# antofuller/jumbo_mae_tpu

Hardware: AMD Instinct MI355X
Metric: pretrain images/sec (whole node) ViT-L/16 224 mask75% at 1/2/4/8 MI355X (higher is better)
Workload: dtype bf16; 1 GPU; model=vit_large_patch16 jumbo-MAE (3 CLS, shared jumbo MLP) + decoder 8x512x16h, global_batch=4096, seq_len=52, decoder_seq_len=199, parallelism=dp1, per_gpu_batch=4096, grad_accum=2, micro_batch=2048, grad_ckpt=False, hip_graph=False, optimizer=adamw(0.9,0.95) wd0.05 warmup-cosine

## Files before the change

### jumbo_mae_tpu_amd/csrc/bindings.cpp

```cpp
#include <torch/extension.h>
#include <c10/hip/HIPStream.h>
#include <hip/hip_runtime.h>

#include <array>
#include <climits>

#include "jm_api.h"

namespace {

hipStream_t stream() { return c10::hip::getCurrentHIPStream().stream(); }

#define CHECK_CUDA(x) TORCH_CHECK((x).is_cuda(), #x " must be a GPU tensor")
#define CHECK_CONTIG(x) TORCH_CHECK((x).is_contiguous(), #x " must be contiguous")
#define CHECK_DT(x, d) TORCH_CHECK((x).scalar_type() == (d), #x " has wrong dtype")

const uint16_t* bf(const torch::Tensor& t) { return reinterpret_cast<const uint16_t*>(t.data_ptr()); }
uint16_t* bfm(torch::Tensor& t) { return reinterpret_cast<uint16_t*>(t.data_ptr()); }
uint16_t* bfp(const torch::Tensor& t) { return reinterpret_cast<uint16_t*>(t.data_ptr()); }
const float* fopt(const c10::optional<torch::Tensor>& t) {
  return t.has_value() && t->defined() ? t->data_ptr<float>() : nullptr;
}
float* fopt_m(c10::optional<torch::Tensor>& t) { return t.has_value() && t->defined() ? t->data_ptr<float>() : nullptr; }

// ... 767 lines not shown
  GemmEpi ep{nullptr, nullptr, N};
  ep.part = out.data_ptr<float>();
  run_nt("gemm_nt_f32", jm_gemm_nt_plan(M, N, K, EPI_PARTIAL, A.stride(0), 1), A, B, ep);
  return out;
}

torch::Tensor gemm_nt_dgelu(torch::Tensor A, torch::Tensor B, torch::Tensor pre, c10::optional<torch::Tensor> dbias,
                            bool deriv, double rate) {
  CHECK_DT(pre, deriv ? torch::kUInt8 : torch::kBFloat16);
  const auto [M, N, K] = check_nt_operands("gemm_nt_dgelu", A, B);
  TORCH_CHECK(pre.is_contiguous() && pre.size(0) == M && pre.size(1) == N, "gemm_nt_dgelu: pre [M,N]");
  auto out = torch::empty({M, N}, A.options());
  GemmEpi ep{nullptr, bfm(out), N};
  if (deriv) {
    ep.dqa = pre.data_ptr<uint8_t>();
    ep.dqs = (rate > 0.0 ? keep_params(rate).second : 1.f) / GD_Q;
  } else {
    ep.aux = bf(pre);
  }
  GemmPlan plan = jm_gemm_nt_plan(M, N, K, deriv ? EPI_DMUL : EPI_DGELU, A.stride(0), 1);
  float* db = bias_ptr("gemm_nt_dgelu dbias", dbias, N);
  torch::Tensor part;
  if (db) {
    const auto f32 = A.options().dtype(torch::kFloat32);
    part = plan.colpart_zero ? torch::zeros({plan.colpart_rows, N}, f32) : torch::empty({plan.colpart_rows, N}, f32);
    ep.colpart = part.data_ptr<float>();
  } else {
    plan.colpart = false;
  }
  run_nt("gemm_nt_dgelu", plan, A, B, ep);
  if (db) check_rc(jm_splitk_reduce_add(part.data_ptr<float>(), db, N, plan.colpart_rows, stream()),
                   "gemm_nt_dgelu dbias");
  return out;
}

py::dict gemm_nt_plan_dict(int M, int N, int K, int epi, long lda, int splits) {
  const GemmPlan p = jm_gemm_nt_plan(M, N, K, epi, lda, splits);
  using namespace py::literals;
  return py::dict("status"_a = p.status, "family"_a = p.family, "tile_rows"_a = p.tile_rows,
                  "tile_cols"_a = p.tile_cols, "row_tiles"_a = p.row_tiles, "col_tiles"_a = p.col_tiles,
                  "tiles"_a = p.tiles, "grid"_a = p.grid, "tail_S"_a = p.tail_S, "tail_r"_a = p.tail_r,
                  "tail_floats"_a = p.tail_floats, "colpart"_a = p.colpart, "colpart_rows"_a = p.colpart_rows,
                  "colpart_zero"_a = p.colpart_zero);
}

torch::Tensor rrc_resize(torch::Tensor src, torch::Tensor tab, int64_t size, int64_t tmp_bytes, int64_t tmp_rows_max) {
  CHECK_CUDA(src);
  CHECK_CUDA(tab);
  CHECK_DT(src, torch::kUInt8);
  CHECK_DT(tab, torch::kInt64);
  TORCH_CHECK(src.dim() == 1 && src.is_contiguous(), "rrc_resize: src must be a flat uint8 buffer");
  TORCH_CHECK(tab.dim() == 2 && tab.size(1) == 13 && tab.is_contiguous(), "rrc_resize: tab [B, 13] int64");
  TORCH_CHECK(size > 0 && size <= 4096 && tmp_bytes > 0 && tmp_rows_max > 0, "rrc_resize: bad sizes");
  const int B = tab.size(0);
  auto out = torch::empty({B, 3, size, size}, src.options());
  auto tmp = torch::empty({tmp_bytes}, src.options());
  check_rc(jm_rrc_resize(src.data_ptr<uint8_t>(), tab.data_ptr<int64_t>(), B, (int)size, tmp.data_ptr<uint8_t>(),
                         (int)tmp_rows_max, out.data_ptr<uint8_t>(), stream()),
           "rrc_resize");
  return out;
}

torch::Tensor window_resize(torch::Tensor src, torch::Tensor tab, int64_t size, int64_t tmp_bytes,
                            int64_t tmp_rows_max) {
  CHECK_CUDA(src);
  CHECK_CUDA(tab);
// ... 1177 lines not shown
  m.def("attn_dropout", &attn_dropout, py::arg("S"), py::arg("hd"));
  m.def("gemm_tn_wgrad", &gemm_tn_wgrad, py::arg("dy"), py::arg("x"), py::arg("g"), py::arg("store") = false);
  m.def("gemm_tn_wgrad_seg", &gemm_tn_wgrad_seg, py::arg("dys"), py::arg("xs"), py::arg("g"), py::arg("store") = false);
  m.def("zero_ranges", &zero_ranges, "zero float ranges of a flat buffer (one launch)");
  m.def("colsum_add_f32", &colsum_add_f32, "g += x.sum(0) for a row-strided fp32 [rows, n] view");
  m.def("gemm_tn_wgrad_seg_group", &gemm_tn_wgrad_seg_group, py::arg("dys"), py::arg("xs"), py::arg("gs"),
        py::arg("stores") = std::vector<bool>{}, "grouped segmented weight gradients (<= 2 problems)");
  m.def("gemm_tn_wgrad_group", &gemm_tn_wgrad_group, py::arg("dys"), py::arg("xs"), py::arg("gs"),
        py::arg("stores") = std::vector<bool>{}, "grouped weight gradients over one M (<= 4 problems)");
  m.def("gemm_test_force", &jm_gemm_test_force, py::arg("path"), py::arg("rows") = 0,
        "numerics tests only: NT GEMM kernel path 0 = by shape, 1 = 64-deep main loop everywhere, "
        "2 = 4-phase kernels at every M without tail split (rows = forced tile height)");
  m.def("gemm_nt_plan", &gemm_nt_plan_dict, py::arg("M"), py::arg("N"), py::arg("K"), py::arg("epi") = 0,
        py::arg("lda") = 0, py::arg("splits") = 1,
        "the launch plan of an NT GEMM (csrc/gemm_plan.h GemmPlan) as a dict; read-only");
  m.def(
      "gemm_nt_tiles", [](int M, int N, int K, int epi, long lda) { return jm_gemm_nt_plan(M, N, K, epi, lda, 1).tiles; },
      py::arg("M"), py::arg("N"), py::arg("K") = 1024, py::arg("epi") = 0, py::arg("lda") = 0,
      "output tiles (workgroups before split-K) of an NT launch");
  m.def(
      "gemm_nt_tail_plan",
      [](int M, int N, int K, int epi, long lda) {
        const GemmPlan p = jm_gemm_nt_plan(M, N, K, epi, lda, 1);
        return std::make_pair(p.tail_S, p.tail_r);
      },
      py::arg("M"), py::arg("N"), py::arg("K"), py::arg("epi") = 0, py::arg("lda") = 0,
      "(S, tail tiles) of the tail split of an NT launch (S = 0: none); read-only");
  m.def("transpose_bf16_batch", &transpose_bf16_batch);
  m.def("gemm_nt_splitk", &gemm_nt_splitk, py::arg("A"), py::arg("B"), py::arg("bias") = py::none(),
        py::arg("splits") = 8, py::arg("add") = py::none());
  m.def("gemm_nt_dgelu", &gemm_nt_dgelu, py::arg("A"), py::arg("B"), py::arg("pre"), py::arg("dbias") = py::none(),
        py::arg("deriv") = false, py::arg("rate") = 0.0);
  m.def("gemm_nt_f32", &gemm_nt_f32, py::arg("A"), py::arg("B"));
  m.def("gemm_nt", &gemm_nt, py::arg("A"), py::arg("B"), py::arg("bias") = py::none(), py::arg("gelu") = false,
        py::arg("gelu_only") = false, py::arg("gelu_deriv") = false, py::arg("seed") = py::none(),
        py::arg("rate") = 0.0);
  m.def("opt_sumsq", &opt_sumsq);
  m.def("opt_adamw", &opt_adamw);
  m.def("opt_lamb_phase1", &opt_lamb_phase1);
  m.def("opt_lars_norms", &opt_lars_norms);
  m.def("opt_apply_trust", &opt_apply_trust);
  m.def("opt_sgd", &opt_sgd);
  m.def("opt_ema", &opt_ema, py::arg("master"), py::arg("ema"), py::arg("rows"), py::arg("meta"),
        py::arg("ema_hyper"));
  m.def("ema_swap", &ema_swap, py::arg("master"), py::arg("ema"), py::arg("shadow"), py::arg("rows"));
  m.def("opt_seg_stats", &opt_seg_stats, py::arg("master"), py::arg("grad"), py::arg("p_old"), py::arg("rows"),
        py::arg("meta"), py::arg("out") = py::none());
  m.def("patchify_normalize", &patchify_normalize);
  m.def("gather_patches", &gather_patches);
  m.def("embed_finish", &embed_finish);
  m.def("zero_f32", &zero_f32, "fp32 zero fill kernel (the store-mode gradients' pre-reduce fill)");
  m.def("mask_ids", &mask_ids, "random-masking permutation ids + mask from noise (one workgroup per row)");
  m.def("unshuffle_fwd", &unshuffle_fwd);
  m.def("unshuffle_bwd", &unshuffle_bwd);
  m.def("patch_mse_fwd", &patch_mse_fwd);
  m.def("mix_patches", &mix_patches);
  m.def("patch_mse_bwd", &patch_mse_bwd);
  m.def("recon", &recon, py::arg("pred"), py::arg("images"), py::arg("mask"), py::arg("p"), py::arg("norm_pix"),
        py::arg("fill") = 127, py::arg("out") = py::none(),
        "MAE reconstruction panels -> (recon, paste, masked uint8 [B, 3, H, W], err fp32 [B, N])");
  m.def("cls_loss_fwd", &cls_loss_fwd, py::arg("logits"), py::arg("labels"), py::arg("perm") = py::none(),
        py::arg("w") = py::none(), py::arg("smoothing") = 0.0, py::arg("mode") = 0);
  m.def("cls_loss_bwd", &cls_loss_bwd, py::arg("dloss"), py::arg("logits"), py::arg("labels"),
        py::arg("perm"), py::arg("w"), py::arg("smoothing"), py::arg("mode"), py::arg("lse"));
  m.def("kd_loss_fwd", &kd_loss_fwd, py::arg("z"), py::arg("u"), py::arg("temperature") = 1.0, py::arg("mode") = 0,
        "distillation loss -> (kd fp32 [B], agree bool [B], lse fp32 [B, 4], t int32 [B])");
// ... 65 lines not shown
```

### jumbo_mae_tpu_amd/csrc/gemm.hip

```cpp
#include <type_traits>

#include "common.h"
#include "jm_api.h"

namespace {

constexpr int BM = 256, BN = 256;
constexpr size_t GEMM_SMEM = 128 * 1024;

typedef __attribute__((address_space(3))) void lds_void_t;

JM_DEVICE __amdgpu_buffer_rsrc_t make_rsrc(const uint16_t* base, long bytes) {
  const int n = bytes >= 0xffffffffL ? -1 : (int)bytes;
  return __builtin_amdgcn_make_buffer_rsrc((void*)base, (short)0, n, 0x00020000);
}

JM_DEVICE void blds16(__amdgpu_buffer_rsrc_t r, uint32_t voff, uint32_t soff, uint16_t* l) {
  __builtin_amdgcn_raw_ptr_buffer_load_lds(r, (lds_void_t*)(l), 16, voff, soff, 0, 0);
}

JM_DEVICE bf16x8_t lds8(const uint16_t* p) { return *reinterpret_cast<const bf16x8_t*>(p); }

JM_DEVICE f32x4_t mfma16(bf16x8_t a, bf16x8_t b, f32x4_t c) {
  return __builtin_amdgcn_mfma_f32_16x16x32_bf16(a, b, c, 0, 0, 0);
// ... 51 lines not shown
            gd_put<3>(dv[3], gd_put<2>(dv[2], gd_put<1>(dv[1], gd_put<0>(dv[0], 0u))));
        store4(ep.out2 + (long)m * ep.ldo + n, gv);
        continue;
      }
      store4(ep.out + (long)m * ep.ldo + n, v);
      if (EPI == EPI_GELU) {
        float gv[4];
#pragma unroll
        for (int i = 0; i < 4; ++i) gv[i] = gelu_tanh_f(bf2f(f2bf(v[i])));
        store4(ep.out2 + (long)m * ep.ldo + n, gv);
      }
    }
  }
}

template <int BNT = BN, int TR = BM>
JM_DEVICE void tile_of(int M, int N, int GROUP_M, int& m0, int& n0, int splits = 1, int* split = nullptr) {
  const int nM = (M + TR - 1) / TR, nN = (N + BNT - 1) / BNT;
  const int nwg = nM * nN * splits;
  const int orig = blockIdx.x;
  const int xcd = orig & 7, q = nwg >> 3, r = nwg & 7;
  int wg = (xcd < r ? xcd * (q + 1) : r * (q + 1) + (xcd - r) * q) + (orig >> 3);
  if (split) {
    *split = wg / (nM * nN);
    wg -= *split * (nM * nN);
  }
  const int per_group = GROUP_M * nN;
  const int first_m = (wg / per_group) * GROUP_M;
  const int gsz = min(nM - first_m, GROUP_M);
  m0 = (first_m + (wg % per_group) % gsz) * TR;
  n0 = ((wg % per_group) / gsz) * BNT;
}

JM_DEVICE void tile_coords(int g, int M, int N, int GROUP_M, int& m0, int& n0) {
  const int nM = (M + BM - 1) / BM, nN = (N + BN - 1) / BN;
  const int per_group = GROUP_M * nN;
  const int first_m = (g / per_group) * GROUP_M;
  const int gsz = min(nM - first_m, GROUP_M);
  m0 = (first_m + (g % per_group) % gsz) * BM;
  n0 = ((g % per_group) / gsz) * BN;
}

JM_DEVICE void tile_of_range(int M, int N, int GROUP_M, int t_begin, int t_count, int splits, int& m0, int& n0,
                             int& split, int& tg) {
  const int nwg = t_count * splits;
  const int orig = blockIdx.x;
  const int xcd = orig & 7, q = nwg >> 3, r = nwg & 7;
  int wg = (xcd < r ? xcd * (q + 1) : r * (q + 1) + (xcd - r) * q) + (orig >> 3);
  split = wg / t_count;
  tg = wg - split * t_count;
  tile_coords(t_begin + tg, M, N, GROUP_M, m0, n0);
}

template <typename T>
JM_DEVICE void st16(T* p, uint4 v, bool nts) {
  typedef __attribute__((ext_vector_type(4))) unsigned int u32x4_t;
  if (nts) __builtin_nontemporal_store(u32x4_t{v.x, v.y, v.z, v.w}, reinterpret_cast<u32x4_t*>(p));
  else *reinterpret_cast<uint4*>(p) = v;
}

JM_DEVICE void st8(uint8_t* p, uint2 v, bool nts) {
  typedef __attribute__((ext_vector_type(2))) unsigned int u32x2_t;
  if (nts) __builtin_nontemporal_store(u32x2_t{v.x, v.y}, reinterpret_cast<u32x2_t*>(p));
  else *reinterpret_cast<uint2*>(p) = v;
}

JM_DEVICE uint4 pack8(const float* f) {
  uint4 v;
  v.x = pack_bf2(f[0], f[1]);
  v.y = pack_bf2(f[2], f[3]);
  v.z = pack_bf2(f[4], f[5]);
  v.w = pack_bf2(f[6], f[7]);
// ... 488 lines not shown
  } else if (N % 8 == 0)
    epilogue_lds<EPI, NTW, 512, BN, true, 2 * HR>(acc, ep, smem, M, N, m0, n0, wr, wc, l16, g);
  else
    epilogue<EPI, NTW, MTW>(acc, ep, M, N, m0 + wr * HR, n0 + wc * NTW * 16, l16, g);
}

template <int EPI, int MTL = 4>
__global__ __launch_bounds__(512, 1) void gemm_p4_kernel(const uint16_t* __restrict__ A, long lda,
                                                         const uint16_t* __restrict__ B, long ldb, int M, int N,
                                                         int K, GemmEpi ep, int GROUP_M) {
  JM_DGUARD(blockDim.x == 512 && K % 128 == 0 && M > 0 && N > 0);
  extern __shared__ __attribute__((aligned(16))) uint16_t smem[];
  if (__builtin_amdgcn_readfirstlane(threadIdx.x) >= 256) __builtin_amdgcn_s_setprio(1);
  int m0, n0, split = 0;
  if (EPI != EPI_PARTIAL && ep.t_count > 0) {
    int tg;
    tile_of_range(M, N, GROUP_M, ep.t_begin, ep.t_count, 1, m0, n0, split, tg);
  } else {
    tile_of<BN, 128 + 32 * MTL>(M, N, GROUP_M, m0, n0, EPI == EPI_PARTIAL ? ep.splits : 1,
                                EPI == EPI_PARTIAL ? &split : nullptr);
  }
  int k_begin = 0;
  if (EPI == EPI_PARTIAL) {
    const int ku = K / 128;
    const int ku0 = split * ku / ep.splits, ku1 = (split + 1) * ku / ep.splits;
    k_begin = ku0 * 128;
    K = (ku1 - ku0) * 128;
  }
  f32x4_t acc[8][4];
  p4_mainloop<MTL>(A, lda, B, ldb, M, N, m0, n0, k_begin, K, acc, smem);
  p4_epilogue<EPI, MTL>(acc, ep, M, N, m0, n0, split, smem);
}

constexpr int NBM = 128, NBN = 192, NKT = 64;
constexpr int N_AEL = NBM * NKT, N_BEL = NBN * NKT, N_STAGE = N_AEL + N_BEL;
constexpr int N_RING = 3;
constexpr int N_LD = NBN + 8;
static_assert(N_RING * N_STAGE * 2 <= (int)GEMM_SMEM, "narrow ring exceeds the LDS budget");

JM_DEVICE void narrow_tile(int M, int N, int GROUP_M, int splits, int& m0, int& n0, int& split) {
  const int nM = (M + NBM - 1) / NBM, nN = (N + NBN - 1) / NBN;
  const int tiles = nM * nN, nwg = tiles * splits;
  const int orig = blockIdx.x;
  const int xcd = orig & 7, q = nwg >> 3, r = nwg & 7;
  int wg = (xcd < r ? xcd * (q + 1) : r * (q + 1) + (xcd - r) * q) + (orig >> 3);
  split = wg / tiles;
  wg -= split * tiles;
  const int per_group = GROUP_M * nN;
  const int first_m = (wg / per_group) * GROUP_M;
  const int gsz = min(nM - first_m, GROUP_M);
  m0 = (first_m + (wg % per_group) % gsz) * NBM;
  n0 = ((wg % per_group) / gsz) * NBN;
}

template <int EPI>
JM_DEVICE void narrow_epilogue(const f32x4_t (&acc)[4][3], const GemmEpi& ep, uint16_t* cs, int M, int N, int m0,
                               int n0, int split, int wr, int wc, int l16, int g) {
  if constexpr (EPI == EPI_PARTIAL) {
    float* dst = ep.part + (long)split * M * N;
#pragma unroll
    for (int mt = 0; mt < 4; ++mt) {
      const int m = m0 + wr * 64 + mt * 16 + l16;
      if (m >= M) continue;
#pragma unroll
      for (int nt = 0; nt < 3; ++nt) {
        const int n = n0 + wc * 48 + nt * 16 + 4 * g;
// ... 330 lines not shown
  g_test_path = (path == 1 || path == 2) ? path : 0;
  g_test_rows = (g_test_path == 2 && (rows == 224 || rows == 192 || rows == 160 || rows == 256)) ? rows : 0;
}

GemmPlan jm_gemm_nt_plan(int M, int N, int K, int epi, long lda, int splits) {
  return gemm_nt_plan(M, N, K, epi, lda, splits, num_cus(), g_test_path, g_test_rows);
}

int jm_gemm_nt(const GemmPlan& p, const uint16_t* A, const uint16_t* B, long ldb, const GemmEpi& ep, hipStream_t st) {
  if (p.status) return p.status;
  if ((long)p.N * ldb * 2 >= (1L << 32)) return -2;
  if ((p.tail_S && ep.tail == nullptr) || p.colpart != (ep.colpart != nullptr)) return -5;
  return with_epi(p.epi, [&](auto e) {
    constexpr int EPI = decltype(e)::value;
    GemmEpi em = ep;
    em.splits = p.splits;
    em.tail_S = p.tail_S;
    em.t_begin = 0;
    em.t_count = p.tail_S ? p.grid : 0;
    launch_main<EPI>(p, A, B, ldb, em, st);
    if constexpr (gemm_tail_epi(EPI)) {
      if (p.tail_S) {
        GemmEpi et = em;
        et.t_begin = p.grid;
        et.t_count = p.tail_r;
        launch<gemm_nt64_kernel<EPI_TAIL, false>>(GEMM_SMEM, p.tail_r * p.tail_S, p, A, B, ldb, et, st);
        tail_finish_kernel<EPI><<<p.tail_r * GEMM_PLAN_TAIL_BANDS, 256, 0, st>>>(et, p.M, p.N, GEMM_GROUP);
      }
    }
    return 0;
  });
}

JM_DEBUG_EXPORT(gemm)
```

### jumbo_mae_tpu_amd/csrc/gemm_plan.h

```cpp
#pragma once
#include <initializer_list>

enum { EPI_STORE = 0, EPI_GELU = 1, EPI_DGELU = 2, EPI_PARTIAL = 3, EPI_GELU_ONLY = 4, EPI_TAIL = 5, EPI_GELU_D = 6,
       EPI_DMUL = 7 };

enum { GEMM_NARROW = 0,
       GEMM_P4 = 1,
       GEMM_NT64 = 2 };

constexpr int GEMM_PLAN_BM = 256, GEMM_PLAN_BN = 256, GEMM_PLAN_NBM = 128, GEMM_PLAN_NBN = 192;
constexpr int GEMM_PLAN_TAIL_BANDS = 8;

constexpr bool gemm_tail_epi(int epi) {
  return epi == EPI_STORE || epi == EPI_GELU || epi == EPI_DGELU || epi == EPI_GELU_ONLY;
}

struct GemmPlan {
  int status;
  int M, N, K, epi, splits;
  long lda;
  int family;
  int tile_rows, tile_cols;
  int row_tiles, col_tiles, tiles;
  int grid;
// ... 48 lines not shown
    if (S > K / 512) S = K / 512;
    if (S > 8) S = 8;
    if (S < 2) S = 0, r = 0;
  }

  int rows = BM;
  if (!narrow && deep && !splitk && (long)M * lda * 2 < (1L << 31) - (1L << 20)) {
    if (force_rows) {
      rows = force_rows;
    } else {
      float best_c = S ? (t256 / ncu + 0.8f) * BM : (float)cdiv(t256, ncu) * BM;
      for (int tr : {224, 192, 160}) {
        const float c = (float)cdiv(cdiv(M, tr) * nN, ncu) * tr * gemm_rows_cost(tr);
        if (c < best_c) best_c = c, rows = tr;
      }
    }
  }
  if (rows != BM) S = 0, r = 0;

  p.family = narrow ? GEMM_NARROW : (deep && (epi != EPI_PARTIAL || K / 128 >= splits) ? GEMM_P4 : GEMM_NT64);
  p.tile_rows = narrow ? NBM : rows;
  p.tile_cols = narrow ? NBN : BN;
  p.row_tiles = (int)cdiv(M, p.tile_rows);
  p.col_tiles = (int)cdiv(N, p.tile_cols);
  p.tiles = p.row_tiles * p.col_tiles;
  p.grid = epi == EPI_PARTIAL ? p.tiles * splits : p.tiles - r;
  p.tail_S = S, p.tail_r = r;
  p.tail_floats = (long)S * r * BM * BN;
  p.colpart = colsum;
  p.colpart_rows = p.row_tiles + GEMM_PLAN_TAIL_BANDS * r;
  p.colpart_zero = r > 0;
  return p;
}
```

### jumbo_mae_tpu_amd/csrc/jm_api.h

```cpp
#pragma once
#include <cstddef>
#include <cstdint>

#include <hip/hip_runtime.h>

#include "gemm_plan.h"

struct JmDrop {
  const int64_t* seed;
  uint32_t thr;
  float scale;
  long ioff;
};

struct JmLnRes {
  const uint16_t* y;
  uint16_t* dy;
  long yB, yT;
  const float* scale;
  const float* mask;
  int T0;
  float* dscale;
  float* dbias;
  JmDrop drop;
// ... 8 lines not shown
  int tile0[5];
  int n;
};

struct TnSegs {
  const uint16_t* a[64];
  const uint16_t* b[64];
  int rows;
  int n;
};

constexpr float GD_Q = 195.f;
constexpr int GD_Z = 34;

struct GemmEpi {
  const float* bias;
  uint16_t* out;
  long ldo;
  uint16_t* out2;
  const uint16_t* aux;
  float* colpart;
  float* part;
  int splits;
  float* tail;
  int tail_S;
  int t_begin;
  int t_count;
  const int64_t* dseed;
  uint32_t dthr;
  float dscale;
  uint8_t* dq;
  const uint8_t* dqa;
  float dqs;
};


int jm_layernorm_fwd(const float* x, long sB, long sT, int B, int T, int D, const float* gamma, const float* beta,
                     float eps, void* y, int out_bf16, float* mean, float* rstd, hipStream_t st, uint16_t* y2 = nullptr);
int jm_layernorm_bwd(const void* dy, int dy_bf16, const float* x, long sB, long sT, int B, int T, int D,
                     const float* mean, const float* rstd, const float* gamma, float* dx_ptr, long oB, long oT,
                     const float* dres, long rB, long rT, float* dgamma, float* dbeta, int accum_params, float* ws,
                     const JmLnRes* res, hipStream_t st, const uint16_t* hx = nullptr,
                     const float* beta = nullptr);
int jm_layernorm_bwd_blocks(int rows, int D);
int jm_residual_ln_fwd(const float* x, long sB, long sT, const uint16_t* y, const float* scale, const float* mask,
                       float* x1, long oB, long oT, uint16_t* h, float* mean, float* rstd, int B, int T, int T0,
                       int D, const float* gamma, const float* beta, float eps, hipStream_t st, int R0 = 0,
                       JmDrop drop = JmDrop{nullptr, 0u, 1.f, 0});
int jm_debug_line_layernorm();

int jm_gelu_fwd(const uint16_t* h, uint16_t* a, long n, hipStream_t st);
long jm_rowcol_ws_floats(int M, int N, int nacc);
int jm_gelu_bwd(const uint16_t* h, const uint16_t* da, uint16_t* dh, float* bias_grad, int M, int N, hipStream_t st,
                int deriv, float* ws);
int jm_colsum_bf16(const uint16_t* x, float* acc, int M, int N, hipStream_t st, float* ws);
int jm_residual_fwd(const float* x, long sB, long sT, int B, int T, int D, const uint16_t* y, const float* scale,
                    const float* mask, float* out, long oB, long oT, hipStream_t st, JmDrop drop);
int jm_residual_bwd(const float* dout, long dB, long dT, const uint16_t* y, const float* scale, const float* mask,
                    float* dscale, uint16_t* dy, int B, int T, int D, float* dbias, long yB, long yT, hipStream_t st,
                    JmDrop drop, float* ws);
void jm_zero_f32(float* p, long n, hipStream_t st);
int jm_splitk_reduce_add(const float* part, float* g, long n, int S, hipStream_t st, int store = 0);
int jm_colsum_add_f32(const float* x, long ld, int rows, long n, float* g, hipStream_t st);
int jm_zero_ranges(float* base, const long long* desc, int n, long long blocks, hipStream_t st);
int jm_transpose_bf16(const uint16_t* src, uint16_t* dst, int R, int C, hipStream_t st);
int jm_transpose_bf16_batch(const long long* desc, int n, int tiles, hipStream_t st);
// ... 37 lines not shown
void jm_ema_swap(float* p, float* ema, uint16_t* shadow, const int* chunks, int nchunks, long n, hipStream_t st);
constexpr int JM_SEG_STATS_COLS = 7;
void jm_opt_seg_stats(const float* p, const float* g, const float* p_old, const int* chunks, int nchunks,
                      const float* meta, int nseg, long n, double* part, double* out, hipStream_t st);
int jm_debug_line_optim();

int jm_patchify_normalize(const uint8_t* img, float* out, int B, int H, int W, int p, hipStream_t st);
int jm_gather_patches(const uint8_t* img, const int* ids, long idsB, uint16_t* out, int B, int K, int H, int W, int p,
                      hipStream_t st);
int jm_embed_finish(const uint16_t* e, const float* pos, const int* ids, long idsB, const float* cls, float* out,
                    int B, int C, int K, int D, hipStream_t st);
int jm_mask_ids(const float* noise, int R, int N, int keep, int64_t* shuffle, int64_t* restore, int* keep32,
                int* restore32, float* mask, hipStream_t st);
int jm_unshuffle_fwd(const uint16_t* y, const float* tok, const int* restore, long rsB, const float* pos, float* out,
                     int B, int C, int K, int N, int d, hipStream_t st);
int jm_unshuffle_bwd_blocks(int B, int C, int N, int rows_per_block);
int jm_unshuffle_bwd(const float* dout, const int* restore, long rsB, uint16_t* dy, double* part, int B, int C, int K,
                     int N, int d, int rows_per_block, hipStream_t st);
int jm_mix_patches(const uint8_t* img, const int* perm, const float* prm, const int* box, uint16_t* out, int B, int H,
                   int W, int p, hipStream_t st);
int jm_patch_mse_fwd(const uint16_t* pred, long ldp, const uint8_t* img, float* mse, long rows, int N, int H, int W,
                     int p, int norm_pix, hipStream_t st);
int jm_patch_mse_bwd(const uint16_t* pred, long ldp, const uint8_t* img, const float* dmse, uint16_t* dpred, long rows,
                     int N, int H, int W, int p, int norm_pix, hipStream_t st);
int jm_debug_line_mae();

int jm_recon(const void* pred, int pred_bf16, const uint8_t* img, const float* mask, long maskB, uint8_t* recon,
             uint8_t* paste, uint8_t* masked, float* err, int B, int H, int W, int p, int norm_pix, int fill,
             hipStream_t st);
int jm_debug_line_recon();

GemmPlan jm_gemm_nt_plan(int M, int N, int K, int epi, long lda, int splits);
int jm_gemm_nt(const GemmPlan& plan, const uint16_t* A, const uint16_t* B, long ldb, const GemmEpi& ep, hipStream_t st);
void jm_gemm_test_force(int path, int rows);
int jm_debug_line_gemm();

size_t jm_gemm_tn_smem();
int jm_gemm_tn_plan(const TnGroup& grp, int M, int* S_out);
int jm_gemm_tn(const TnGroup& grp, const TnSegs* segs, int M, int sps, int S, hipStream_t st, int store);
int jm_debug_line_gemm_tn();

int jm_dropout_apply(const void* x, void* y, long n, int bf16, const int64_t* seed, uint32_t thr, float scale,
                     hipStream_t st);
int jm_gelu_drop(const uint16_t* h, uint16_t* g, uint16_t* gp, long n, const int64_t* seed, uint32_t thr, float scale,
                 hipStream_t st);
int jm_softmax_dropout_fwd(const float* z, float* p, float* pd, long rows, int S, const int64_t* seed, uint32_t thr,
                           float scale, hipStream_t st);
int jm_softmax_dropout_bwd(const float* dpd, const float* p, float* dz, long rows, int S, const int64_t* seed,
                           uint32_t thr, float scale, hipStream_t st);
int jm_debug_line_dropout();

int jm_rrc_resize(const uint8_t* src, const int64_t* tab, int B, int S, uint8_t* tmp, int tmp_rows_max, uint8_t* out,
                  hipStream_t st);
int jm_window_resize(const uint8_t* src, const int64_t* tab, int B, int S, uint8_t* tmp, int tmp_rows_max,
                     uint8_t* out, hipStream_t st);
int jm_window_tab();
int jm_rrc_kmax();
int jm_debug_line_augment();

int jm_aug_stat_words();
int jm_aug_record_len();
int jm_aug_chain(uint8_t* images, uint8_t* scratch, const double* chain, int B, int slots, int S, uint32_t* stats,
                 hipStream_t st);
int jm_augmix_mix(const uint8_t* orig, const uint8_t* chains, const float* table, uint8_t* out, int B, int W, int S,
                  int blended, hipStream_t st);
int jm_erase_paste(uint8_t* images, const int64_t* table, const uint8_t* fill, long fill_len, int B, int S,
// ... 89 lines not shown
```

### jumbo_mae_tpu_amd/ops/blocks.py

```python

from __future__ import annotations


import torch

from typing import NamedTuple

from . import attn_maps as AM
from . import attn_stats as AS
from . import dropout as Dr
from . import prims as P


LINKS = True
FWD_LINKS = True


class Link:

    __slots__ = ("spec", "dy", "done", "dx_key", "ln1", "h1")

    def __init__(self, ln1=None):
        self.spec = None
        self.dy = None
# ... 44 lines not shown
    if AS._COLLECTOR is not None:
        AS.observe(qkv.view(B, S, -1), attn.heads)
    if AM._COLLECTOR is not None:
        AM.observe(qkv.view(B, S, -1), attn.heads)
    o, lse = P.attn_fwd(qkv.view(B, S, -1), attn.heads, drop=(dr.attn, dr.rate) if dr is not None else None)
    a = P.linear_fwd(o.view(B * S, -1), attn.wo_k, attn.wo_b)
    return qkv, o, lse, a, qs


def _od(dr: Drops | None, name: str, base):
    return None if dr is None else (getattr(dr, name), dr.rate, base)


def _attn_bwd(attn, da, h1, qkv, o, lse, B, S, wo_bias_done=False, dr: Drops | None = None, rope=None, qs=None):
    do = P.linear_bwd(da, o.view(B * S, -1), attn.wo_k, attn.wo_b, bias_done=wo_bias_done)
    plain = rope is None and qs is None
    dqkv, bd = P.attn_bwd(do, qkv.view(B, S, -1), o, lse, attn.heads, attn.qkv_b if plain else None,
                          drop=(dr.attn, dr.rate) if dr is not None else None)
    if qs is not None:
        dqkv, dg = P.qknorm_bwd_(dqkv.view(B, S, -1), qs, attn.heads, attn.q_norm.master, attn.k_norm.master, rope)
        attn.q_norm.accumulate_grad(dg[0])
        attn.k_norm.accumulate_grad(dg[1])
    elif rope is not None:
        dqkv = P.rope_(dqkv.view(B, S, -1), attn.heads, rope.n_cls, rope.gw, rope.table, rope.pos, inverse=True)
    return P.linear_bwd(dqkv.view(B * S, -1), h1, attn.qkv_k, attn.qkv_b, bias_done=bd)


def _ff_fwd(ff, h, train=True, rate=0.0, sh=None, so=None):
    if ff.kind == "swiglu":
        pre = P.linear_fwd(h, ff.w13.k, ff.w13.b)
        a = P.swiglu_fwd(pre, (sh, rate) if sh is not None else None)
        y = P.linear_fwd(a, ff.w2.k, ff.w2.b)
        return pre, a, y, False
    pre, g, deriv, dropped = P.linear_gelu_fwd_saved(h, ff.w1.k, ff.w1.b, need_pre=train,
                                                     drop=(sh, rate) if sh is not None else None)
    if sh is not None and not dropped:
        g, pre = Dr.gelu_drop(pre, None, sh, rate)
        deriv = True
    y = P.linear_fwd(g, ff.w2.k, ff.w2.b)
    return pre, g, y, deriv


def _ff_bwd(ff, dy, h, pre, g, w2_bias_done=False, dx_add=None, deriv=False, rate=0.0, sh=None):
    if ff.kind == "swiglu":
        da = P.linear_bwd(dy, g, ff.w2.k, ff.w2.b, bias_done=w2_bias_done)
        hb13 = ff.w13.b if ff.w13.k.segs[0].trainable else None
        dpre, bias_done = P.swiglu_bwd(pre, da, hb13, (sh, rate) if sh is not None else None)
        return P.linear_bwd(dpre, h, ff.w13.k, ff.w13.b, bias_done=bias_done, dx_add=dx_add)
    hb1 = ff.w1.b if ff.w1.k.segs[0].trainable else None
    dpre, bias_done = P.linear_gelu_bwd(dy, g, pre, ff.w2.k, ff.w2.b, hb1, w2_bias_done, deriv, rate)
    return P.linear_bwd(dpre, h, ff.w1.k, ff.w1.b, bias_done=bias_done, dx_add=dx_add)


def _note_uses(*handles):
    for h in handles:
        if h is not None:
            h.note_use()


def _attn_handles(attn):
    return (attn.qkv_k, attn.qkv_b, attn.wo_k, attn.wo_b, attn.q_norm, attn.k_norm)


def _ff_handles(ff):
    if ff.kind == "swiglu":
        return (ff.w13.k, ff.w13.b, ff.w2.k, ff.w2.b)
    return (ff.w1.k, ff.w1.b, ff.w2.k, ff.w2.b)


class JumboBlockFn(torch.autograd.Function):
    @staticmethod
    def forward(ctx, x, anchor, layer, m1, m2, m3, link_in, link_out, train=True, dr=None, rope=None):
        B, S, D = x.shape
        C = layer.C
        J = C * D
        dt = layer.norm1.g.store.compute_dtype
        h1, mu1, rs1 = _ln1_fwd(x, layer, link_in, dt)
        qkv, o, lse, a, qs = _attn_fwd(layer.attn, h1, B, S, dr, rope)
        x1, hp, mup, rsp = P.residual_ln_fwd(x, a, layer.scale1, m1, layer.norm2.g, layer.norm2.b, C,
                                             drop=_od(dr, "wo", a))
        cls_in = x1[:, :C].reshape(B, 1, J)
        hc, muc, rsc, hcb = P.ln_fwd(cls_in, layer.norm3.g, layer.norm3.b, torch.float32, dt)
        rate = dr.rate if dr is not None else 0.0
        jpre, jg, jy, jd = _ff_fwd(layer.jumbo_mlp, hcb, train, rate, dr and dr.jh, dr and dr.jo)
        pin = x1[:, C:]
        fpre, fg, fy, fd = _ff_fwd(layer.ff, hp, train, rate, dr and dr.fh, dr and dr.fo)
        x2 = torch.empty_like(x1)
        P.residual_fwd(hc.view(B, 1, J), jy, layer.scale3, m3, out=x2[:, :C].reshape(B, 1, J), drop=_od(dr, "jo", jy))
        nl = link_out.ln1 if link_out is not None else None
        if nl is not None:
            _, h1n, mun, rsn = P.residual_ln_fwd(x1, fy, layer.scale2, m2, nl[0], nl[1], 0, C, out=x2,
                                                 drop=_od(dr, "fo", fy))
            link_out.put_h1(x2, h1n, mun, rsn)
        else:
            P.residual_fwd(pin, fy, layer.scale2, m2, out=x2[:, C:], drop=_od(dr, "fo", fy))
        ctx.save_for_backward(x, mu1, rs1, h1, qkv, o, lse, a, x1, muc, rsc, hcb, jpre, jg, jy,
                              hp, mup, rsp, fpre, fg, fy, m1, m2, m3, qs)
        ctx.layer = layer
        ctx.link_in, ctx.link_out = link_in, link_out
        ctx.gelu_deriv = (jd, fd)
        ctx.gelu_rate = rate
        ctx.dr = dr
        ctx.rope = rope
        if link_out is not None:
            link_out.spec = P.ResSpec(fy, layer.scale2, m2, layer.ff.w2.b, C, drop=_od(dr, "fo", fy))
        return x2

    @staticmethod
    def backward(ctx, dx2):
        with P.paired_wgrads():
            dx = _jumbo_bwd(ctx, dx2)
        return dx, None, None, None, None, None, None, None, None, None, None


def _jumbo_bwd(ctx, dx2):
    (x, mu1, rs1, h1, qkv, o, lse, a, x1, muc, rsc, hcb, jpre, jg, jy,
     hp, mup, rsp, fpre, fg, fy, m1, m2, m3, qs) = ctx.saved_tensors
    layer = ctx.layer
    dr = ctx.dr
# ... 119 lines not shown
```

### jumbo_mae_tpu_amd/ops/prims.py

```python

from __future__ import annotations

import contextlib
import math
import os

from typing import NamedTuple

import torch
import torch.nn.functional as F

from ..models.params import Handle
from . import _ext
from . import qknorm as QN
from . import swiglu as SG
from .rope import rope_torch

LN_EPS = 1e-6
_GELU_C = math.sqrt(2.0 / math.pi)


def hip(t: torch.Tensor) -> bool:
    return _ext.use_hip(t)

# ... 97 lines not shown

_GEMM_MODE = "auto"
_DGRAD_OURS = True
_CLS_LOSS_OURS = True
_KD_OURS = True
_EVAL_REPORT_OURS = True
_BN_OURS = True
_KNN_OURS = True
_FEAT_STATS_OURS = True
_NORMS_OURS = True
_ATTN_STATS_OURS = True
_ATTN_MAPS_OURS = True
_ROPE_OURS = True
_QKNORM_OURS = True
_SWIGLU_OURS = True


NARROW_MAX_M = 4096
_NARROW_FUSED_MIN_TILES = 160


def nt_tiles(M: int, N: int) -> int:
    if M < NARROW_MAX_M:
        return -(-M // 128) * -(-N // 192)
    return -(-M // 256) * -(-N // 256)


def use_our_gemm(M: int, N: int, K: int, fused_gelu: bool = False) -> bool:
    if _GEMM_MODE == "blas" or K % 64 or N % 8:
        return False
    if M >= NARROW_MAX_M:
        return True
    return not fused_gelu or nt_tiles(M, N) >= _NARROW_FUSED_MIN_TILES


def splitk_plan(M: int, N: int, K: int) -> int:
    if _GEMM_MODE == "blas" or M >= NARROW_MAX_M or K % 64 or N % 8:
        return 0
    if nt_tiles(M, N) >= _NARROW_FUSED_MIN_TILES:
        return 0
    s = min(256 // nt_tiles(M, N), K // 512, 16)
    return s if s >= 2 else 0


def _pad_cols(t: torch.Tensor, mult: int = 64) -> torch.Tensor:
    c = t.shape[1]
    pad = -c % mult
    return F.pad(t, (0, pad)) if pad else t.contiguous()


def linear_fwd(x2: torch.Tensor, hw: Handle, hb: Handle | None) -> torch.Tensor:
    w = hw.weight()
    if hip(x2) and x2.dtype == torch.bfloat16:
        s = splitk_plan(x2.shape[0], w.shape[0], x2.shape[1])
        if s:
            return _ext.load().gemm_nt_splitk(x2, w, hb.master if hb is not None else None, s)
    if hip(x2) and x2.dtype == torch.bfloat16 and use_our_gemm(x2.shape[0], w.shape[0], x2.shape[1]):
        return _ext.load().gemm_nt(x2, w, hb.master if hb is not None else None, False)[0]
    if hb is not None:
        return torch.addmm(hb.weight(), x2, w.t())
    return x2 @ w.t()


def linear_gelu_fwd(x2: torch.Tensor, hw: Handle, hb: Handle | None, need_pre: bool = True):
    w = hw.weight()
    if hip(x2) and x2.dtype == torch.bfloat16 and use_our_gemm(x2.shape[0], w.shape[0], x2.shape[1], True):
# ... 577 lines not shown
```

Before: 6652 images/sec.

## Run jumbo-MLP and patch-MLP GEMMs together in one grouped NT launch

Adds a grouped GEMM kernel that runs two independent NT problems, the small jumbo CLS MLP and the large per-patch MLP, in a single launch with one shared tile size and an XCD-aware workgroup remap. Both the first (GELU-derivative) and second (store) FFN GEMMs in the block forward go through it when one problem is below the narrow-M threshold and the other is above. The aim is to fill the GPU with the small jumbo GEMM's tiles alongside the large one instead of running an under-occupied launch on its own. The cost is a single row-tile size for both problems and extra epilogue selection per workgroup.

```diff
diff --git a/jumbo_mae_tpu_amd/csrc/bindings.cpp b/jumbo_mae_tpu_amd/csrc/bindings.cpp
--- a/jumbo_mae_tpu_amd/csrc/bindings.cpp
+++ b/jumbo_mae_tpu_amd/csrc/bindings.cpp
@@ -823,6 +823,102 @@
   if (db) check_rc(jm_splitk_reduce_add(part.data_ptr<float>(), db, N, plan.colpart_rows, stream()),
                    "gemm_nt_dgelu dbias");
   return out;
+}
+
+using OptTensors = std::vector<c10::optional<torch::Tensor>>;
+std::vector<torch::Tensor> gemm_nt_group(std::vector<torch::Tensor> A, std::vector<torch::Tensor> B, OptTensors bias,
+                                         int64_t epi, OptTensors aux, OptTensors dbias, OptTensors seed, double rate,
+                                         OptTensors out, OptTensors out2) {
+  TORCH_CHECK(A.size() == 2 && B.size() == 2, "gemm_nt_group: two problems");
+  TORCH_CHECK(epi == EPI_STORE || epi == EPI_GELU_D || epi == EPI_DMUL, "gemm_nt_group: epilogue");
+  const auto opt = [](const OptTensors& v, int p, const char* what) -> const torch::Tensor* {
+    TORCH_CHECK(v.empty() || v.size() == 2, "gemm_nt_group: ", what, " must be empty or have two entries");
+    return !v.empty() && v[p].has_value() && v[p]->defined() ? &*v[p] : nullptr;
+  };
+  NtGroup grp{};
+  std::vector<torch::Tensor> res, part(2);
+  for (int p = 0; p < 2; ++p) {
+    const auto [M, N, K] = check_nt_operands("gemm_nt_group", A[p], B[p]);
+    TORCH_CHECK(epi == EPI_STORE || N % 8 == 0, "gemm_nt_group: N % 8 == 0 with a fused epilogue");
+    NtProblem& q = grp.p[p];
+    q.A = bf(A[p]), q.B = bf(B[p]), q.lda = A[p].stride(0), q.ldb = B[p].stride(0), q.M = M, q.N = N, q.K = K;
+    const auto first_dt = epi == EPI_GELU_D ? torch::kUInt8 : torch::kBFloat16;
+    const auto given = [&](const torch::Tensor* t, c10::ScalarType dt, const char* what) {
+      if (t == nullptr) return torch::empty({M, N}, A[p].options().dtype(dt));
+      TORCH_CHECK(t->is_cuda() && t->scalar_type() == dt && t->dim() == 2 && t->size(0) == M && t->size(1) == N &&
+                      t->stride(1) == 1 && t->stride(0) >= N && t->stride(0) % 8 == 0 &&
+                      reinterpret_cast<uintptr_t>(t->data_ptr()) % 16 == 0,
+                  "gemm_nt_group: ", what, " must be [M, N] with unit column stride and 16-byte aligned rows");
+      return *t;
+    };
+    torch::Tensor o1 = given(opt(out, p, "out"), first_dt, "out");
+    q.ep.ldo = o1.stride(0);
+    q.ep.splits = 1;
+    if (const torch::Tensor* b = opt(bias, p, "bias")) {
+      TORCH_CHECK(epi != EPI_DMUL, "gemm_nt_group: EPI_DMUL takes no bias");
+      q.ep.bias = bias_ptr("gemm_nt_group bias", *b, N);
+    }
+    res.push_back(o1);
+    if (epi == EPI_GELU_D) {
+      torch::Tensor o2 = given(opt(out2, p, "out2"), torch::kBFloat16, "out2");
+      TORCH_CHECK(o2.stride(0) == o1.stride(0), "gemm_nt_group: out and out2 of a problem share the row stride");
+      q.ep.dq = o1.data_ptr<uint8_t>();
+      q.ep.out2 = bfm(o2);
+      res.push_back(o2);
+      const torch::Tensor* s = opt(seed, p, "seed");
+      if (s != nullptr && rate > 0.0) {
+        check_seed(*s, A[p]);
+        const auto kp = keep_params(rate);
+        q.ep.dseed = s->data_ptr<int64_t>();
+        q.ep.dthr = kp.first;
+        q.ep.dscale = kp.second;
+      }
+    } else {
+      q.ep.out = bfm(o1);
+    }
+    if (epi == EPI_DMUL) {
+      const torch::Tensor* a = opt(aux, p, "aux");
+      TORCH_CHECK(a != nullptr && a->is_cuda() && a->scalar_type() == torch::kUInt8 && a->dim() == 2 &&
+                      a->size(0) == M && a->size(1) == N && a->stride(1) == 1 && a->stride(0) == o1.stride(0),
+                  "gemm_nt_group: aux = uint8 gelu' codes [M, N] with the output's row stride");
+      q.ep.dqa = a->data_ptr<uint8_t>();
+      q.ep.dqs = (rate > 0.0 ? keep_params(rate).second : 1.f) / GD_Q;
+    }
+  }
+  const GemmGroupPlan plan = jm_gemm_nt_group_plan(grp, (int)epi);
+  TORCH_CHECK(plan.status == 0, "gemm_nt_group: unsupported launch (status ", plan.status, ")");
+  if (epi == EPI_DMUL) {
+    for (int p = 0; p < 2; ++p) {
+      if (opt(dbias, p, "dbias") == nullptr) continue;
+      const int rows = plan.colpart_rows[p == plan.first ? 0 : 1];
+      part[p] = torch::empty({rows, grp.p[p].N}, A[p].options().dtype(torch::kFloat32));
+      grp.p[p].ep.colpart = part[p].data_ptr<float>();
+    }
+  }
+  check_rc(jm_gemm_nt_group(plan, grp, stream()), "gemm_nt_group");
+  if (epi == EPI_DMUL) {
+    for (int p = 0; p < 2; ++p) {
+      const torch::Tensor* d = opt(dbias, p, "dbias");
+      if (d == nullptr) continue;
+      float* db = bias_ptr("gemm_nt_group dbias", *d, grp.p[p].N);
+      check_rc(jm_splitk_reduce_add(part[p].data_ptr<float>(), db, grp.p[p].N, (int)part[p].size(0), stream()),
+               "gemm_nt_group dbias");
+    }
+  }
+  return res;
+}
+
+py::dict gemm_nt_group_plan_dict(std::vector<int> M, std::vector<int> N, std::vector<int> K, std::vector<long> lda,
+                                 int epi) {
+  TORCH_CHECK(M.size() == 2 && N.size() == 2 && K.size() == 2 && lda.size() == 2, "gemm_nt_group_plan: two problems");
+  NtGroup grp{};
+  for (int p = 0; p < 2; ++p) grp.p[p].M = M[p], grp.p[p].N = N[p], grp.p[p].K = K[p], grp.p[p].lda = lda[p];
+  const GemmGroupPlan g = jm_gemm_nt_group_plan(grp, epi);
+  using namespace py::literals;
+  const auto two = [](const int* v) { return py::make_tuple(v[0], v[1]); };
+  return py::dict("status"_a = g.status, "first"_a = g.first, "tile_rows"_a = g.tile_rows,
+                  "row_tiles"_a = two(g.row_tiles), "col_tiles"_a = two(g.col_tiles), "tiles"_a = two(g.tiles),
+                  "grid"_a = g.grid, "colpart_rows"_a = two(g.colpart_rows));
 }
 
 py::dict gemm_nt_plan_dict(int M, int N, int K, int epi, long lda, int splits) {
@@ -2066,6 +2162,12 @@
   m.def("gemm_nt_dgelu", &gemm_nt_dgelu, py::arg("A"), py::arg("B"), py::arg("pre"), py::arg("dbias") = py::none(),
         py::arg("deriv") = false, py::arg("rate") = 0.0);
   m.def("gemm_nt_f32", &gemm_nt_f32, py::arg("A"), py::arg("B"));
+  m.def("gemm_nt_group", &gemm_nt_group, py::arg("A"), py::arg("B"), py::arg("bias") = OptTensors{}, py::arg("epi") = 0,
+        py::arg("aux") = OptTensors{}, py::arg("dbias") = OptTensors{}, py::arg("seed") = OptTensors{},
+        py::arg("rate") = 0.0, py::arg("out") = OptTensors{}, py::arg("out2") = OptTensors{},
+        "two NT problems with one epilogue kind (0 store, 6 gelu' codes + gelu, 7 dmul) in one launch");
+  m.def("gemm_nt_group_plan", &gemm_nt_group_plan_dict, py::arg("M"), py::arg("N"), py::arg("K"), py::arg("lda"),
+        py::arg("epi") = 0, "the plan of a grouped NT launch (csrc/gemm_plan.h GemmGroupPlan) as a dict; read-only");
   m.def("gemm_nt", &gemm_nt, py::arg("A"), py::arg("B"), py::arg("bias") = py::none(), py::arg("gelu") = false,
         py::arg("gelu_only") = false, py::arg("gelu_deriv") = false, py::arg("seed") = py::none(),
         py::arg("rate") = 0.0);
diff --git a/jumbo_mae_tpu_amd/csrc/gemm.hip b/jumbo_mae_tpu_amd/csrc/gemm.hip
--- a/jumbo_mae_tpu_amd/csrc/gemm.hip
+++ b/jumbo_mae_tpu_amd/csrc/gemm.hip
@@ -107,12 +107,13 @@
   n0 = ((wg % per_group) / gsz) * BNT;
 }
 
+template <int TR = BM>
 JM_DEVICE void tile_coords(int g, int M, int N, int GROUP_M, int& m0, int& n0) {
-  const int nM = (M + BM - 1) / BM, nN = (N + BN - 1) / BN;
+  const int nM = (M + TR - 1) / TR, nN = (N + BN - 1) / BN;
   const int per_group = GROUP_M * nN;
   const int first_m = (g / per_group) * GROUP_M;
   const int gsz = min(nM - first_m, GROUP_M);
-  m0 = (first_m + (g % per_group) % gsz) * BM;
+  m0 = (first_m + (g % per_group) % gsz) * TR;
   n0 = ((g % per_group) / gsz) * BN;
 }
 
@@ -667,6 +668,50 @@
   p4_epilogue<EPI, MTL>(acc, ep, M, N, m0, n0, split, smem);
 }
 
+JM_DEVICE GemmEpi pick_epi(bool s, const GemmEpi& a, const GemmEpi& b) {
+  GemmEpi e;
+  e.bias = s ? b.bias : a.bias;
+  e.out = s ? b.out : a.out;
+  e.ldo = s ? b.ldo : a.ldo;
+  e.out2 = s ? b.out2 : a.out2;
+  e.aux = s ? b.aux : a.aux;
+  e.colpart = s ? b.colpart : a.colpart;
+  e.part = nullptr;
+  e.splits = 1;
+  e.tail = nullptr;
+  e.tail_S = 0;
+  e.t_begin = 0;
+  e.t_count = 0;
+  e.dseed = s ? b.dseed : a.dseed;
+  e.dthr = s ? b.dthr : a.dthr;
+  e.dscale = s ? b.dscale : a.dscale;
+  e.dq = s ? b.dq : a.dq;
+  e.dqa = s ? b.dqa : a.dqa;
+  e.dqs = s ? b.dqs : a.dqs;
+  return e;
+}
+
+template <int EPI, int MTL>
+__global__ __launch_bounds__(512, 1) void gemm_p4_group_kernel(NtGroup grp, int tiles0, int GROUP_M) {
+  JM_DGUARD(blockDim.x == 512 && tiles0 > 0 && tiles0 < (int)gridDim.x);
+  extern __shared__ __attribute__((aligned(16))) uint16_t smem[];
+  if (__builtin_amdgcn_readfirstlane(threadIdx.x) >= 256) __builtin_amdgcn_s_setprio(1);
+  int wg = gemm_group_remap((int)blockIdx.x, tiles0, (int)gridDim.x);
+  const bool s = wg >= tiles0;
+  if (s) wg -= tiles0;
+  const NtProblem &pa = grp.p[0], &pb = grp.p[1];
+  const uint16_t* A = s ? pb.A : pa.A;
+  const uint16_t* B = s ? pb.B : pa.B;
+  const long lda = s ? pb.lda : pa.lda, ldb = s ? pb.ldb : pa.ldb;
+  const int M = s ? pb.M : pa.M, N = s ? pb.N : pa.N, K = s ? pb.K : pa.K;
+  const GemmEpi ep = pick_epi(s, pa.ep, pb.ep);
+  int m0, n0;
+  tile_coords<128 + 32 * MTL>(wg, M, N, GROUP_M, m0, n0);
+  f32x4_t acc[8][4];
+  p4_mainloop<MTL>(A, lda, B, ldb, M, N, m0, n0, 0, K, acc, smem);
+  p4_epilogue<EPI, MTL>(acc, ep, M, N, m0, n0, 0, smem);
+}
+
 constexpr int NBM = 128, NBN = 192, NKT = 64;
 constexpr int N_AEL = NBM * NKT, N_BEL = NBN * NKT, N_STAGE = N_AEL + N_BEL;
 constexpr int N_RING = 3;
@@ -1063,4 +1108,51 @@
   });
 }
 
+GemmGroupPlan jm_gemm_nt_group_plan(const NtGroup& grp, int epi) {
+  const int M[2] = {grp.p[0].M, grp.p[1].M}, N[2] = {grp.p[0].N, grp.p[1].N}, K[2] = {grp.p[0].K, grp.p[1].K};
+  const long lda[2] = {grp.p[0].lda, grp.p[1].lda};
+  return gemm_nt_group_plan(M, N, K, lda, epi, num_cus(), g_test_path == 2 ? g_test_rows : 0);
+}
+
+namespace {
+
+template <int EPI, int MTL>
+void launch_group(const GemmGroupPlan& p, const NtGroup& g, hipStream_t st) {
+  static bool attr = false;
+  if (!attr) {
+    (void)hipFuncSetAttribute((const void*)gemm_p4_group_kernel<EPI, MTL>, hipFuncAttributeMaxDynamicSharedMemorySize,
+                              (int)GEMM_SMEM);
+    attr = true;
+  }
+  gemm_p4_group_kernel<EPI, MTL><<<p.grid, 512, GEMM_SMEM, st>>>(g, p.tiles[0], GEMM_GROUP);
+}
+
+}
+
+int jm_gemm_nt_group(const GemmGroupPlan& p, const NtGroup& grp, hipStream_t st) {
+  if (p.status) return p.status;
+  if (p.tiles[0] <= 0 || p.tiles[1] <= 0) return -1;
+  NtGroup g;
+  g.p[0] = grp.p[p.first];
+  g.p[1] = grp.p[1 - p.first];
+  for (int i = 0; i < 2; ++i) {
+    if ((long)g.p[i].N * g.p[i].ldb * 2 >= (1L << 32)) return -2;
+    if (g.p[i].A == nullptr || g.p[i].B == nullptr) return -1;
+  }
+  const auto go = [&](auto e) {
+    constexpr int EPI = decltype(e)::value;
+    if (p.tile_rows == 224) launch_group<EPI, 3>(p, g, st);
+    else if (p.tile_rows == 192) launch_group<EPI, 2>(p, g, st);
+    else if (p.tile_rows == 160) launch_group<EPI, 1>(p, g, st);
+    else launch_group<EPI, 4>(p, g, st);
+    return 0;
+  };
+  switch (p.epi) {
+    case EPI_STORE: return go(std::integral_constant<int, EPI_STORE>{});
+    case EPI_GELU_D: return go(std::integral_constant<int, EPI_GELU_D>{});
+    case EPI_DMUL: return go(std::integral_constant<int, EPI_DMUL>{});
+  }
+  return -3;
+}
+
 JM_DEBUG_EXPORT(gemm)
diff --git a/jumbo_mae_tpu_amd/csrc/gemm_plan.h b/jumbo_mae_tpu_amd/csrc/gemm_plan.h
--- a/jumbo_mae_tpu_amd/csrc/gemm_plan.h
+++ b/jumbo_mae_tpu_amd/csrc/gemm_plan.h
@@ -104,3 +104,66 @@
   p.colpart_zero = r > 0;
   return p;
 }
+
+
+constexpr bool gemm_group_epi(int epi) { return epi == EPI_STORE || epi == EPI_GELU_D || epi == EPI_DMUL; }
+
+constexpr int gemm_group_remap(int orig, int tiles0, int nwg) {
+  const int x = orig & 7, s = orig >> 3;
+  const int q0 = tiles0 >> 3, r0 = tiles0 & 7, Q = nwg >> 3, R = nwg & 7;
+  const int base0 = x * q0 + (x < r0 ? x : r0);
+  const int mine0 = q0 + (x < r0 ? 1 : 0);
+  if (s < mine0) return base0 + s;
+  const int base = x * Q + (x < R ? x : R);
+  return tiles0 + (base - base0) + (s - mine0);
+}
+
+struct GemmGroupPlan {
+  int status;
+  int epi;
+  int first;
+  int tile_rows;
+  int row_tiles[2], col_tiles[2], tiles[2];
+  int grid;
+  int colpart_rows[2];
+};
+
+inline GemmGroupPlan gemm_nt_group_plan(const int M[2], const int N[2], const int K[2], const long lda[2], int epi,
+                                        int ncu, int force_rows) {
+  GemmGroupPlan g{};
+  g.epi = epi;
+  if (ncu < 1) ncu = 1;
+  const auto cdiv = [](long a, long b) { return (a + b - 1) / b; };
+  bool short_ok = true;
+  for (int p = 0; p < 2; ++p) {
+    if (K[p] <= 0 || K[p] % 128 || N[p] % 4 || M[p] <= 0 || N[p] <= 0) g.status = g.status ? g.status : -1;
+    else if ((long)M[p] * lda[p] * 2 >= (1L << 32)) g.status = g.status ? g.status : -2;
+    if ((long)M[p] * lda[p] * 2 >= (1L << 31) - (1L << 20)) short_ok = false;
+  }
+  if (!g.status && (!gemm_group_epi(epi) || ((epi == EPI_GELU_D || epi == EPI_DMUL) && (N[0] % 8 || N[1] % 8))))
+    g.status = -3;
+  g.first = K[1] > K[0] || (K[1] == K[0] && cdiv(M[1], GEMM_PLAN_BM) * cdiv(N[1], GEMM_PLAN_BN) <
+                                                 cdiv(M[0], GEMM_PLAN_BM) * cdiv(N[0], GEMM_PLAN_BN));
+  const int o[2] = {g.first, 1 - g.first};
+  int rows = GEMM_PLAN_BM;
+  if (force_rows == 256 || force_rows == 224 || force_rows == 192 || force_rows == 160) {
+    rows = short_ok ? force_rows : GEMM_PLAN_BM;
+  } else if (short_ok && !g.status) {
+    float best = 0.f;
+    for (int tr : {256, 224, 192, 160}) {
+      float work = 0.f;
+      for (int p = 0; p < 2; ++p) work += (float)(cdiv(M[p], tr) * cdiv(N[p], GEMM_PLAN_BN)) * (float)K[p];
+      const float c = (work / ncu + (float)K[o[1]]) * tr * gemm_rows_cost(tr);
+      if (tr == 256 || c < best) best = c, rows = tr;
+    }
+  }
+  g.tile_rows = rows;
+  for (int p = 0; p < 2; ++p) {
+    g.row_tiles[p] = M[o[p]] > 0 ? (int)cdiv(M[o[p]], rows) : 0;
+    g.col_tiles[p] = N[o[p]] > 0 ? (int)cdiv(N[o[p]], GEMM_PLAN_BN) : 0;
+    g.tiles[p] = g.row_tiles[p] * g.col_tiles[p];
+    g.colpart_rows[p] = g.row_tiles[p];
+  }
+  g.grid = g.tiles[0] + g.tiles[1];
+  return g;
+}
diff --git a/jumbo_mae_tpu_amd/csrc/jm_api.h b/jumbo_mae_tpu_amd/csrc/jm_api.h
--- a/jumbo_mae_tpu_amd/csrc/jm_api.h
+++ b/jumbo_mae_tpu_amd/csrc/jm_api.h
@@ -64,6 +64,17 @@
   uint8_t* dq;
   const uint8_t* dqa;
   float dqs;
+};
+
+struct NtProblem {
+  const uint16_t* A;
+  const uint16_t* B;
+  long lda, ldb;
+  int M, N, K;
+  GemmEpi ep;
+};
+struct NtGroup {
+  NtProblem p[2];
 };
 
 
@@ -167,6 +178,8 @@
 
 GemmPlan jm_gemm_nt_plan(int M, int N, int K, int epi, long lda, int splits);
 int jm_gemm_nt(const GemmPlan& plan, const uint16_t* A, const uint16_t* B, long ldb, const GemmEpi& ep, hipStream_t st);
+GemmGroupPlan jm_gemm_nt_group_plan(const NtGroup& grp, int epi);
+int jm_gemm_nt_group(const GemmGroupPlan& plan, const NtGroup& grp, hipStream_t st);
 void jm_gemm_test_force(int path, int rows);
 int jm_debug_line_gemm();
 
diff --git a/jumbo_mae_tpu_amd/ops/blocks.py b/jumbo_mae_tpu_amd/ops/blocks.py
--- a/jumbo_mae_tpu_amd/ops/blocks.py
+++ b/jumbo_mae_tpu_amd/ops/blocks.py
@@ -100,13 +100,36 @@
         a = P.swiglu_fwd(pre, (sh, rate) if sh is not None else None)
         y = P.linear_fwd(a, ff.w2.k, ff.w2.b)
         return pre, a, y, False
+    pre, g, deriv = _ff1_fwd(ff, h, train, rate, sh)
+    y = P.linear_fwd(g, ff.w2.k, ff.w2.b)
+    return pre, g, y, deriv
+
+
+def _ff1_fwd(ff, h, train, rate, sh):
     pre, g, deriv, dropped = P.linear_gelu_fwd_saved(h, ff.w1.k, ff.w1.b, need_pre=train,
                                                      drop=(sh, rate) if sh is not None else None)
     if sh is not None and not dropped:
         g, pre = Dr.gelu_drop(pre, None, sh, rate)
         deriv = True
-    y = P.linear_fwd(g, ff.w2.k, ff.w2.b)
-    return pre, g, y, deriv
+    return pre, g, deriv
+
+
+def _ff_fwd_pair(ffa, ha, sha, ffb, hb, shb, train=True, rate=0.0):
+    if not train or not P._GELU_DERIV or ffa.kind == "swiglu" or ffb.kind == "swiglu":
+        return _ff_fwd(ffa, ha, train, rate, sha), _ff_fwd(ffb, hb, train, rate, shb)
+    if P.group_nt_ok((ha, hb), (ffa.w1.k.weight(), ffb.w1.k.weight()), "ff1"):
+        (qa, ga), (qb, gb) = P.linear_gelu_fwd_saved_pair(
+            (ha, hb), (ffa.w1.k, ffb.w1.k), (ffa.w1.b, ffb.w1.b),
+            ((sha, rate) if sha is not None else None, (shb, rate) if shb is not None else None))
+        da = db = True
+    else:
+        qa, ga, da = _ff1_fwd(ffa, ha, train, rate, sha)
+        qb, gb, db = _ff1_fwd(ffb, hb, train, rate, shb)
+    if P.group_nt_ok((ga, gb), (ffa.w2.k.weight(), ffb.w2.k.weight()), "ff2"):
+        ya, yb = P.linear_fwd_pair((ga, gb), (ffa.w2.k, ffb.w2.k), (ffa.w2.b, ffb.w2.b))
+    else:
+        ya, yb = P.linear_fwd(ga, ffa.w2.k, ffa.w2.b), P.linear_fwd(gb, ffb.w2.k, ffb.w2.b)
+    return (qa, ga, ya, da), (qb, gb, yb, db)
 
 
 def _ff_bwd(ff, dy, h, pre, g, w2_bias_done=False, dx_add=None, deriv=False, rate=0.0, sh=None):
@@ -150,9 +173,9 @@
         cls_in = x1[:, :C].reshape(B, 1, J)
         hc, muc, rsc, hcb = P.ln_fwd(cls_in, layer.norm3.g, layer.norm3.b, torch.float32, dt)
         rate = dr.rate if dr is not None else 0.0
-        jpre, jg, jy, jd = _ff_fwd(layer.jumbo_mlp, hcb, train, rate, dr and dr.jh, dr and dr.jo)
+        (jpre, jg, jy, jd), (fpre, fg, fy, fd) = _ff_fwd_pair(layer.jumbo_mlp, hcb, dr and dr.jh,
+                                                              layer.ff, hp, dr and dr.fh, train, rate)
         pin = x1[:, C:]
-        fpre, fg, fy, fd = _ff_fwd(layer.ff, hp, train, rate, dr and dr.fh, dr and dr.fo)
         x2 = torch.empty_like(x1)
         P.residual_fwd(hc.view(B, 1, J), jy, layer.scale3, m3, out=x2[:, :C].reshape(B, 1, J), drop=_od(dr, "jo", jy))
         nl = link_out.ln1 if link_out is not None else None
diff --git a/jumbo_mae_tpu_amd/ops/prims.py b/jumbo_mae_tpu_amd/ops/prims.py
--- a/jumbo_mae_tpu_amd/ops/prims.py
+++ b/jumbo_mae_tpu_amd/ops/prims.py
@@ -153,6 +153,37 @@
     if M >= NARROW_MAX_M:
         return True
     return not fused_gelu or nt_tiles(M, N) >= _NARROW_FUSED_MIN_TILES
+
+
+GROUP_NT = True
+_GROUP_NT_MIN_M = 512
+
+
+def group_nt_ok(xs, ws, pair: str = "") -> bool:
+    if GROUP_NT not in (True, "force", pair) or _GEMM_MODE == "blas":
+        return False
+    for x, w in zip(xs, ws):
+        if not (hip(x) and x.dtype == torch.bfloat16 and w.dtype == torch.bfloat16 and x.dim() == 2
+                and x.stride(1) == 1 and w.stride(1) == 1 and x.shape[1] % 128 == 0 and w.shape[0] % 8 == 0):
+            return False
+    if GROUP_NT == "force":
+        return True
+    lo, hi = sorted(x.shape[0] for x in xs)
+    return lo >= _GROUP_NT_MIN_M and lo < NARROW_MAX_M <= hi
+
+
+def linear_gelu_fwd_saved_pair(xs, hws, hbs, drops):
+    rate = max((d[1] for d in drops if d is not None), default=0.0)
+    seeds = [d[0] if d is not None else None for d in drops]
+    q0, g0, q1, g1 = _ext.load().gemm_nt_group(list(xs), [h.weight() for h in hws],
+                                               [h.master if h is not None else None for h in hbs], 6,
+                                               seed=seeds, rate=rate)
+    return [(q0, g0), (q1, g1)]
+
+
+def linear_fwd_pair(xs, hws, hbs):
+    return _ext.load().gemm_nt_group(list(xs), [h.weight() for h in hws],
+                                     [h.master if h is not None else None for h in hbs], 0)
 
 
 def splitk_plan(M: int, N: int, K: int) -> int:
```

Result: no change. 6674 images/sec (median of 6 runs) (+0.3%).
